# Cardinal-Cryptography/zk-apps

Hardware: AMD Instinct MI355X
Metric: shielder_withdraw_groth16_proofs_per_sec_2^20_constraints (higher is better)
Workload: dtype int: signed 28-bit limbs in 32-bit words, 64-bit column accumulators (Fr 255-bit / Fq 381-bit Montgomery); 1 GPU; single withdraw-shaped Groth16 proof, N=2^20 (7 Fr NTTs, 4 G1 MSM + 1 G2 MSM of 2^20-1 terms), 1 proof per step per GPU; relation=update_note (withdraw) with Poseidon-5 hashing, chain-padded to N, curve=BLS12-381, independent_proofs_per_rank=171, distinct_witnesses_per_rank=64, fresh_r_s_per_proof=True, proofs_in_flight_per_gpu=3, msm_schedule=A | B1 (over r*z) + L + H reduced together | B2 (G2)

## Files before the change

include/zkmi.h:

```cpp
#ifndef ZKMI_H
#define ZKMI_H
#include <stdint.h>
#ifdef __cplusplus
extern "C" {
#endif

#define ZKMI_OK 0
#define ZKMI_ERR_BAD_ARG (-1)
#define ZKMI_ERR_NON_CANONICAL (-2)
#define ZKMI_ERR_HIP (-3)
#define ZKMI_ERR_NO_DEVICE (-4)
#define ZKMI_ERR_VERIFICATION (-5)
#define ZKMI_ERR_ACCOUNT_UPDATE (-6)
#define ZKMI_ERR_OPERATION_COMBINE (-7)
#define ZKMI_ERR_UNSATISFIED (-8)
#define ZKMI_ERR_RCCL (-9)

typedef struct zkmi_ctx zkmi_ctx;
typedef struct zkmi_bases_g1 zkmi_bases_g1;
typedef struct zkmi_bases_g2 zkmi_bases_g2;
typedef struct zkmi_r1cs zkmi_r1cs;
typedef struct zkmi_pk zkmi_pk;

const char* zkmi_version(void);
// ... 145 lines not shown
#define ZKMI_OP_DEPOSIT 0
#define ZKMI_OP_WITHDRAW 1
#define ZKMI_MAX_TREE_HEIGHT 32
typedef struct {
  zkmi_fr amount, token, user;
  zkmi_fr new_note[3];
  zkmi_fr old_note[3];
  uint32_t tree_height;
  uint8_t path_shape[ZKMI_MAX_TREE_HEIGHT];
  zkmi_fr path[ZKMI_MAX_TREE_HEIGHT];
  zkmi_fr op_priv_user;
  zkmi_fr account[4];
} zkmi_note_update;
int32_t zkmi_update_note_r1cs(uint32_t log_n, int32_t op_kind, zkmi_r1cs** out);
int32_t zkmi_update_note_r1cs_h(uint32_t log_n, int32_t op_kind, uint32_t tree_height, zkmi_r1cs** out);
int32_t zkmi_update_note_witness(uint32_t log_n, int32_t op_kind, const zkmi_note_update* in, uint8_t* out_z,
                                 uint8_t* out_publics);

int32_t zkmi_update_note_witness_batch_dev(zkmi_ctx* ctx, uint32_t log_n, int32_t op_kind, const zkmi_note_update* in,
                                           uint32_t n, void* const* d_z_out, int32_t* out_status);
int32_t zkmi_update_note_witness_values_host(uint32_t log_n, int32_t op_kind, const zkmi_note_update* in, uint8_t* out_z);

int32_t zkmi_groth16_setup(zkmi_ctx* ctx, const zkmi_r1cs* r1cs, const uint8_t toxic[160], zkmi_pk** out_pk,
                           uint8_t* vk_out, uint64_t vk_cap);
int32_t zkmi_ctx_set_group_size(zkmi_ctx* ctx, uint32_t group);
int32_t zkmi_pk_load(zkmi_ctx* ctx, const zkmi_r1cs* r1cs, const uint8_t alpha_g1[96], const uint8_t beta_g1[96],
                     const uint8_t beta_g2[192], const uint8_t delta_g1[96], const uint8_t delta_g2[192],
                     const uint8_t* a_query, const uint8_t* b_g1_query, const uint8_t* b_g2_query,
                     const uint8_t* h_query, const uint8_t* l_query, zkmi_pk** out_pk);
int32_t zkmi_pk_free(zkmi_pk* pk);
int32_t zkmi_pk_shape(const zkmi_pk* pk, uint32_t* n_vars, uint32_t* n_pub, uint32_t* log_n);
int32_t zkmi_pk_export_g1_elems(const zkmi_pk* pk, uint8_t out_beta_g1[96], uint8_t out_delta_g1[96]);
int32_t zkmi_pk_schedule_state(const zkmi_pk* pk, uint64_t out[3]);
int32_t zkmi_pk_export_query(zkmi_ctx* ctx, const zkmi_pk* pk, int32_t which, uint64_t first, uint64_t count, uint8_t* out);
int32_t zkmi_groth16_prove(zkmi_ctx* ctx, const zkmi_pk* pk, const uint8_t* z, const uint8_t r[32], const uint8_t s[32],
                           uint8_t out_proof[192]);
int32_t zkmi_groth16_prove_dev(zkmi_ctx* ctx, const zkmi_pk* pk, const void* d_z, const uint8_t r[32], const uint8_t s[32],
                               uint8_t out_proof[192]);
int32_t zkmi_groth16_prove_batch_dev(zkmi_ctx* ctx, const zkmi_pk* pk, uint32_t n_proofs, const void* const* d_z,
                                     const uint8_t* r, const uint8_t* s, uint8_t* out_proofs);
int32_t zkmi_groth16_prove_batch(zkmi_ctx* ctx, const zkmi_pk* pk, uint32_t n_proofs, const uint8_t* const* z,
                                 const uint8_t* r, const uint8_t* s, uint8_t* out_proofs);
int32_t zkmi_groth16_witness_map(zkmi_ctx* ctx, const zkmi_pk* pk, const uint8_t* z, uint8_t* out_h);
int32_t zkmi_groth16_prove_batch_multi(zkmi_ctx* const* ctxs, const zkmi_pk* const* pks, uint32_t n_dev, uint32_t n_proofs,
                                       const void* const* z, int32_t z_on_device, const uint8_t* r, const uint8_t* s,
                                       uint8_t* out_proofs);

int32_t zkmi_groth16_verify(const uint8_t* vk, uint32_t n_pub, const uint8_t* publics, const uint8_t proof[192]);

typedef struct zkmi_vk zkmi_vk;
int32_t zkmi_vk_prepare(const uint8_t* vk, uint32_t n_pub, zkmi_vk** out);
int32_t zkmi_vk_free(zkmi_vk* vk);

#define ZKMI_PROOF_OK 0
#define ZKMI_PROOF_BAD_ENCODING 1
#define ZKMI_PROOF_NOT_ON_CURVE 2
#define ZKMI_PROOF_NOT_IN_SUBGROUP 3
#define ZKMI_PROOF_BAD_PUBLIC 4
#define ZKMI_PROOF_PAIRING 5
int32_t zkmi_groth16_verify_batch(zkmi_ctx* ctx, const zkmi_vk* vk, uint64_t n, const uint8_t* publics,
                                  const uint8_t* proofs, const uint8_t* weights, uint8_t* out_status,
                                  uint64_t* out_first_bad);
int32_t zkmi_groth16_verify_each(zkmi_ctx* ctx, const zkmi_vk* vk, uint64_t n, const uint8_t* publics,
                                 const uint8_t* proofs, uint8_t* out_status, uint64_t* out_first_bad);

int32_t zkmi_ark_vk_read(const uint8_t* buf, uint64_t len, int32_t compressed, uint8_t* out_vk, uint64_t vk_cap,
// ... 89 lines not shown
```

include/zkmi_testing.h:

```cpp
#ifndef ZKMI_TESTING_H
#define ZKMI_TESTING_H
#include "zkmi.h"
#ifdef __cplusplus
extern "C" {
#endif

int32_t zkmi_bases_g1_synthetic(zkmi_ctx* ctx, uint64_t n, zkmi_bases_g1** out);
int32_t zkmi_bases_g2_synthetic(zkmi_ctx* ctx, uint64_t n, zkmi_bases_g2** out);
int32_t zkmi_bases_g1_synthetic_range(zkmi_ctx* ctx, uint64_t first, uint64_t n, zkmi_bases_g1** out);
int32_t zkmi_bn254_bases_synthetic(zkmi_ctx* ctx, uint64_t n, zkmi_bn_bases** out);

int32_t zkmi_shielder_r1cs(uint32_t log_n, zkmi_r1cs** out);
int32_t zkmi_shielder_witness(uint32_t log_n, uint64_t seed, uint8_t* out_z );
int32_t zkmi_shielder_witness_from_input(uint32_t log_n, const zkmi_update_note_input* in, uint8_t* out_z);

int32_t zkmi_selftest_fq28(uint64_t seed, uint32_t iters, uint32_t* out_mismatches);
int32_t zkmi_selftest_assembly(uint64_t seed, uint32_t iters, uint32_t* out_mismatches);
int32_t zkmi_selftest_host_pool(uint32_t callers, uint32_t jobs, uint32_t* out_mismatches);
int32_t zkmi_selftest_poseidon(int32_t field, uint64_t seed, uint32_t iters, uint32_t* out_mismatches);
int32_t zkmi_selftest_miller_formulas(const uint8_t g1_affine[96], const uint8_t g2_affine[192], uint8_t out_fq12[576]);
int32_t zkmi_selftest_final_exp_formulas(const uint8_t in_fq12[576], uint8_t out_chain[576], uint8_t out_plain[576]);
int32_t zkmi_verify_each_kernel_ms(float out_ms[3]);
int32_t zkmi_verify_batch_phases(double out_ms[7]);
int32_t zkmi_selftest_quad_add(zkmi_ctx* ctx, uint64_t seed, uint32_t n, uint32_t* out_mismatches);
int32_t zkmi_selftest_fp28_ops(zkmi_ctx* ctx, int32_t field, int32_t op, uint32_t n, const int32_t* in, int32_t* out,
                               uint8_t* out_flag);
int32_t zkmi_selftest_ntt_dif_dev(zkmi_ctx* ctx, int32_t field, void* d_data, uint32_t log_n, int32_t post);
int32_t zkmi_selftest_msm_g1_sum2_dev(zkmi_ctx* ctx, const void* d_scalars_a, const void* d_scalars_b, uint64_t n,
                                      const zkmi_bases_g1* bases, uint8_t out_affine[96]);

#ifdef __cplusplus
}
#endif
#endif
```

zk-apps_amd/binding.py:

```python
import ctypes as C
import os

ERR = {
    0: "OK",
    -1: "BAD_ARG",
    -2: "NON_CANONICAL",
    -3: "HIP",
    -4: "NO_DEVICE",
    -5: "VerificationError",
    -6: "AccountUpdateError",
    -7: "OperationCombineError",
    -8: "UNSATISFIED",
    -9: "RCCL",
}
PHASES = {
    "msm_sort": 0,
    "msm_accum_g1": 1,
    "msm_reduce_g1": 2,
    "msm_accum_g2": 3,
    "msm_reduce_g2": 4,
    "ntt": 5,
    "witness": 6,
    "misc": 7,
}
# ... 1005 lines not shown
        self.ctx._chk(fn(self.ctx.h, self.h))
        return self

    def free(self):
        if self.h:
            fn = self.ctx.lib.zkmi_bases_g1_free if self.group == 1 else self.ctx.lib.zkmi_bases_g2_free
            fn(self.h)
            self.h = None


class ProvingKey:
    def __init__(self, ctx, h, r1cs):
        self.ctx, self.h, self.r1cs = ctx, h, r1cs

    def export_query(self, which, first, count):
        w = 192 if which == 2 else 96
        out = (C.c_uint8 * (w * count))()
        self.ctx._chk(self.ctx.lib.zkmi_pk_export_query(self.ctx.h, self.h, C.c_int32(which), C.c_uint64(first), C.c_uint64(count), out))
        return bytes(out)

    def check(self, checks=CHECK_SUBGROUP):
        where = (C.c_uint64 * 2)(NO_INDEX, NO_INDEX)
        rc = self.ctx.lib.zkmi_pk_check(self.ctx.h, self.h, C.c_int32(checks), where)
        if rc == -2:
            return int(where[0]), int(where[1])
        self.ctx._chk(rc)
        return None

    def schedule_state(self):
        out = (C.c_uint64 * 3)()
        self.ctx._chk(self.ctx.lib.zkmi_pk_schedule_state(self.h, out))
        return bool(out[0]), int(out[1]), int(out[2])

    def free(self):
        if self.h:
            self.ctx.lib.zkmi_pk_free(self.h)
            self.h = None
```

zk-apps_amd/csrc/field28_selftest.hip:

```cpp
#include "ctx.hpp"
#include "field28.hpp"
#include "ntt.hpp"

#ifdef ZKMI_TESTING
using namespace zkmi;

namespace {
enum Op : int {
  OP_ADD = 0, OP_SUB, OP_NEG, OP_DBL, OP_CARRY, OP_MUL, OP_SQR, OP_LAZY_MUL, OP_MSM, OP_X3, OP_SSUB_MUL, OP_IS_ZERO,
  OP_FROM_CANON, OP_TO_CANON, OP_INV,
  OP_FQ2_MUL = 15, OP_FQ2_SQR, OP_FQ2_MSM, OP_FQ2_X3,
  OP_P_MUL = 19, OP_P_SQR, OP_P_MSM, OP_P_SSUB, OP_P_IS_ZERO,
  OP_MUL_FIPS = 24, OP_SQR_FIPS, OP_FIPS2, OP_FIPS4,
  OP_COUNT
};
constexpr int N_IN[OP_COUNT] = {2, 2, 1, 1, 2, 2, 1, 4, 6, 3, 3, 1, 1, 1, 1, 4, 2, 8, 6, 4, 2, 8, 4, 2, 2, 1, 4, 8};
constexpr int N_OUT[OP_COUNT] = {1, 1, 1, 1, 1, 1, 1, 1, 1, 1, 2, 0, 1, 1, 1, 2, 2, 2, 2, 2, 2, 2, 4, 0, 1, 1, 1, 1};

template <class F>
ZK_HD F ld(const int32_t* p) {
  F r;
#pragma unroll
  for (int i = 0; i < F::NL; i++) r.l[i] = p[i];
  return r;
}
template <class F>
ZK_HD void st(int32_t* p, const F& v) {
#pragma unroll
  for (int i = 0; i < F::NL; i++) p[i] = v.l[i];
}

template <class P, int OP>
ZK_HD void op_body(const int32_t* in, int32_t* out, uint8_t* flag, uint32_t t) {
  using F = Fp28<P>;
  constexpr int NL = F::NL;
// ... 124 lines not shown
    if (e == hipSuccess && n_flag) e = hipMemcpyAsync(out_flag, d_flag, (size_t)n_flag * n, hipMemcpyDeviceToHost, ctx->stream);
    const hipError_t es = hipStreamSynchronize(ctx->stream);
    if (e == hipSuccess) e = es;
    (void)hipFree(d_in);
    (void)hipFree(d_out);
    (void)hipFree(d_flag);
    return e == hipSuccess ? ZKMI_OK : ctx->hip_fail(e, "fp28 ops self-test");
  }
}

#define ZK_OP_CASE(OP) \
  case OP: return run_op<P, OP>(ctx, n, in, out, out_flag);
template <class P>
int32_t dispatch(zkmi_ctx* ctx, int32_t op, uint32_t n, const int32_t* in, int32_t* out, uint8_t* out_flag) {
  switch (op) {
    ZK_OP_CASE(OP_ADD) ZK_OP_CASE(OP_SUB) ZK_OP_CASE(OP_NEG) ZK_OP_CASE(OP_DBL) ZK_OP_CASE(OP_CARRY) ZK_OP_CASE(OP_MUL)
    ZK_OP_CASE(OP_SQR) ZK_OP_CASE(OP_LAZY_MUL) ZK_OP_CASE(OP_MSM) ZK_OP_CASE(OP_X3) ZK_OP_CASE(OP_SSUB_MUL)
    ZK_OP_CASE(OP_IS_ZERO) ZK_OP_CASE(OP_FROM_CANON) ZK_OP_CASE(OP_TO_CANON) ZK_OP_CASE(OP_INV)
    ZK_OP_CASE(OP_MUL_FIPS) ZK_OP_CASE(OP_SQR_FIPS) ZK_OP_CASE(OP_FIPS2) ZK_OP_CASE(OP_FIPS4)
    default: break;
  }
  if constexpr (std::is_same<P, Fq28Params>::value) {
    switch (op) {
      ZK_OP_CASE(OP_FQ2_MUL) ZK_OP_CASE(OP_FQ2_SQR) ZK_OP_CASE(OP_FQ2_MSM) ZK_OP_CASE(OP_FQ2_X3)
      ZK_OP_CASE(OP_P_MUL) ZK_OP_CASE(OP_P_SQR) ZK_OP_CASE(OP_P_MSM) ZK_OP_CASE(OP_P_SSUB) ZK_OP_CASE(OP_P_IS_ZERO)
      default: break;
    }
  }
  return ZKMI_ERR_BAD_ARG;
}
#undef ZK_OP_CASE

template <class F, class Dom>
int32_t ntt_dif(zkmi_ctx* ctx, Dom* dom, void* d_data, uint32_t log_n, int32_t post) {
  const uint32_t n = 1u << log_n;
  const uint64_t bytes = (uint64_t)n * sizeof(F);
  if (ctx->d_work_cap < bytes) {
    if (ctx->d_work) (void)hipFree(ctx->d_work);
    ctx->d_work = nullptr;
    ctx->d_work_cap = 0;
    ZK_HIP(ctx, hipMalloc(&ctx->d_work, bytes));
    ctx->d_work_cap = bytes;
  }
  F* work = static_cast<F*>(ctx->d_work);
  ZK_HIP(ctx, ntt_from_canonical(static_cast<const uint32_t*>(d_data), work, n, ctx->stream));
  ZK_HIP(ctx, dom->inverse_to_rev(work, post ? dom->rev_coset_n : nullptr, nullptr, ctx->stream));
  ZK_HIP(ctx, ntt_to_canonical(work, static_cast<uint32_t*>(d_data), n, ctx->stream));
  ZK_HIP(ctx, hipStreamSynchronize(ctx->stream));
  return ZKMI_OK;
}
}

extern "C" int32_t zkmi_selftest_fp28_ops(zkmi_ctx* ctx, int32_t field, int32_t op, uint32_t n, const int32_t* in, int32_t* out,
                                          uint8_t* out_flag) {
  if (!in || n == 0 || n > (1u << 20) || op < 0 || op >= OP_COUNT) return ZKMI_ERR_BAD_ARG;
  switch (field) {
    case 0: return dispatch<Fq28Params>(ctx, op, n, in, out, out_flag);
    case 1: return dispatch<Fr28Params>(ctx, op, n, in, out, out_flag);
    case 2: return dispatch<BnFq28Params>(ctx, op, n, in, out, out_flag);
    case 3: return dispatch<BnFr28Params>(ctx, op, n, in, out, out_flag);
    default: return ZKMI_ERR_BAD_ARG;
  }
}

extern "C" int32_t zkmi_selftest_ntt_dif_dev(zkmi_ctx* ctx, int32_t field, void* d_data, uint32_t log_n, int32_t post) {
  ZK_ENTER(ctx);
  if (!d_data || log_n == 0 || log_n > 26 || (field != 1 && field != 3)) return ZKMI_ERR_BAD_ARG;
  hipError_t e;
  if (field == 1) {
    NttDomain* dom = ctx->domain((int)log_n, &e);
    if (!dom) return ctx->hip_fail(e, "ntt domain init");
    return ntt_dif<Fr28>(ctx, dom, d_data, log_n, post);
  }
  NttDomainBn* dom = ctx->domain_bn((int)log_n, &e);
  if (!dom) return ctx->hip_fail(e, "bn254 ntt domain init");
  return ntt_dif<BnFr28>(ctx, dom, d_data, log_n, post);
}
#endif
```

zk-apps_amd/csrc/groth16.hip:

```cpp
#include <stdlib.h>
#include <string.h>
#include <new>
#include <string>
#include <memory>
#include <chrono>
#include <functional>
#include <thread>
#include <vector>
#include "ctx.hpp"
#include "tune.hpp"
#include "host_pool.hpp"
#include "pairing.hpp"
#include "r1cs.hpp"
#include "points.hpp"

namespace zkmi {

template <class T>
__device__ __forceinline__ T ldv(const T* p) {
  T r;
  const uint4* s = reinterpret_cast<const uint4*>(p);
  uint4* d = reinterpret_cast<uint4*>(&r);
#pragma unroll
  for (unsigned i = 0; i < sizeof(T) / 16; i++) d[i] = s[i];
  return r;
}
template <class T>
__device__ __forceinline__ void stv(T* p, const T& v) {
  const uint4* s = reinterpret_cast<const uint4*>(&v);
  uint4* d = reinterpret_cast<uint4*>(p);
#pragma unroll
  for (unsigned i = 0; i < sizeof(T) / 16; i++) d[i] = s[i];
}

struct MatSet {
  const uint32_t* rowptr[3];
  const uint32_t* col[3];
  const Fr28* val[3];
};
constexpr uint32_t MATVEC_LONG_ROW = 1024;
__global__ void __launch_bounds__(256)
k_matvec_long(MatSet ms, const uint32_t* __restrict__ rows, const Fr28* __restrict__ z, Fr28* __restrict__ out_base, uint32_t n, uint32_t n_vars) {
  __shared__ Fr28 part[256];
  const uint32_t m = rows[2 * blockIdx.x], i = rows[2 * blockIdx.x + 1];
  const uint32_t* __restrict__ col = ms.col[m];
  const Fr28* __restrict__ val = ms.val[m];
  z += (size_t)blockIdx.y * n_vars;
  Fr28 acc = Fr28::zero();
  const uint32_t b = ms.rowptr[m][i], e = ms.rowptr[m][i + 1];
  for (uint32_t k = b + threadIdx.x; k < e; k += 256) acc = acc + ld28(val + k) * ld28(z + col[k]);
  part[threadIdx.x] = acc;
  __syncthreads();
  for (int o = 128; o > 0; o >>= 1) {
    if ((int)threadIdx.x < o) part[threadIdx.x] = part[threadIdx.x] + part[threadIdx.x + o];
    __syncthreads();
  }
  if (threadIdx.x == 0) st28(out_base + (size_t)m * gridDim.y * n + (size_t)blockIdx.y * n + i, part[0]);
}

template <int S>
__global__ void __launch_bounds__(256)
k_matvec(MatSet ms, const Fr28* __restrict__ z, Fr28* __restrict__ out_base, uint32_t nc, uint32_t n, uint32_t n_pub,
         uint32_t n_vars) {
  const int m = blockIdx.z;
  const uint32_t* __restrict__ rowptr = ms.rowptr[m];
  const uint32_t* __restrict__ col = ms.col[m];
  const Fr28* __restrict__ val = ms.val[m];
  const int is_a = m == 0;
  Fr28* __restrict__ out = out_base + (size_t)m * gridDim.y * n;
  z += (size_t)blockIdx.y * n_vars;
  out += (size_t)blockIdx.y * n;
  const uint32_t gi = blockIdx.x * blockDim.x + threadIdx.x;
  const uint32_t i = gi / S, lane = gi % S;
  if (i >= n) return;
  Fr28 acc = Fr28::zero();
  if (i < nc) {
    const uint32_t b = rowptr[i], e = rowptr[i + 1];
    if (e - b > MATVEC_LONG_ROW) return;
    for (uint32_t k = b + lane; k < e; k += S) acc = acc + ld28(val + k) * ld28(z + col[k]);
  } else if (is_a && i < nc + n_pub && lane == 0) {
    acc = ld28(z + (i - nc));
  }
  if constexpr (S > 1) {
#pragma unroll
    for (int o = S / 2; o > 0; o >>= 1) {
      Fr28 t;
#pragma unroll
      for (int q = 0; q < Fr28::NL; q++) t.l[q] = __shfl_xor(acc.l[q], o);
      acc = acc + t;
    }
    if (lane != 0) return;
  }
  st28(out + i, acc);
}

__global__ void __launch_bounds__(256)
k_check_sat(const Fr28* __restrict__ a, const Fr28* __restrict__ b, const Fr28* __restrict__ c,
            const Fr28* __restrict__ z, uint32_t nc, uint32_t* __restrict__ flag, uint32_t n, uint32_t n_vars) {
  a += (size_t)blockIdx.y * n;
  b += (size_t)blockIdx.y * n;
  c += (size_t)blockIdx.y * n;
  z += (size_t)blockIdx.y * n_vars;
  const uint32_t i = blockIdx.x * blockDim.x + threadIdx.x;
  bool bad = false;
  if (i < nc) {
    const Fr28 d = (ld28(a + i) * ld28(b + i) - ld28(c + i)) * Fr28::one();
    bad = !d.is_zero();
  }
  if (i == 0) {
    const Fr28 d = (ld28(z) - Fr28::one()) * Fr28::one();
    bad = bad || !d.is_zero();
  }
// ... 85 lines not shown
      Affine<F> p = ldv(table + w * 256 + d);
      acc.madd(p);
    }
  }
  stv(out + i, acc.to_affine());
}

}

using namespace zkmi;

static bool prover_sort_side() { return ZK_TUNE("ZKMI_SORT_SIDE", 0) == 1; }
static uint32_t prover_solo_max_log() {
  const int v = ZK_TUNE("ZKMI_SOLO_MAX_LOG", 19);
  return (uint32_t)(v < 0 ? 0 : v > 28 ? 28 : v);
}
static bool prover_aux_split() { return ZK_TUNE("ZKMI_AUX_SPLIT", 1) != 0; }

static bool same_bucket_set(const MsmPlan& a, const MsmPlan& b) {
  return a.shared == b.shared && a.c == b.c && a.nwin == b.nwin && a.nb == b.nb && a.seg_log == b.seg_log &&
         a.vec_parts == b.vec_parts && a.ndigits == b.ndigits;
}

struct zkmi_pk {
  zkmi_ctx* ctx = nullptr;
  int device = -1;
  uint32_t n_vars = 0, n_pub = 0, nc = 0, log_n = 0;
  uint32_t tree_height = 0;
  uint32_t gmax = 1;
  uint32_t* d_rowptr[3] = {nullptr, nullptr, nullptr};
  uint32_t* d_long_rows = nullptr;
  uint32_t n_long_rows = 0;
  uint32_t* d_col[3] = {nullptr, nullptr, nullptr};
  Fr28* d_val[3] = {nullptr, nullptr, nullptr};
  G1Affine *a_query = nullptr, *b_g1_query = nullptr, *h_query = nullptr, *l_query = nullptr;
  G2Affine* b_g2_query = nullptr;
  Affine<Fq28>*a28 = nullptr, *b1_28 = nullptr, *h28 = nullptr, *h28_rev = nullptr, *l28 = nullptr;
  Affine<Fq2_28>* b2_28 = nullptr;
  bool shared = false;
  Affine<Fq28>*a_tab = nullptr, *b1_tab = nullptr, *l_tab = nullptr, *h_tab = nullptr;
  Affine<Fq2_28>* b2_tab = nullptr;
  G1Affine alpha_g1, beta_g1, delta_g1, a0, b1_0;
  G2Affine beta_g2, delta_g2, b2_0;
  std::unique_ptr<FixedBase8<Fq>> delta1_tab, k1_tab;
  std::unique_ptr<FixedBase8<Fq2>> delta2_tab;
  G1Affine ka;
  G2Affine kb2;
  Fr* d_z[zkmi_ctx::PROOF_RING] = {};
  mutable const Fr* z_cur[zkmi_ctx::PROOF_RING] = {};
  uint32_t* d_rz[zkmi_ctx::PROOF_RING] = {};
  uint32_t* d_h[zkmi_ctx::PROOF_RING] = {};
  Fr28 *d_zm = nullptr, *d_a = nullptr;
  uint32_t* h_unsat = nullptr;
  uint32_t* h_zent = nullptr;
  mutable bool fold_dense = true;
  mutable uint64_t last_entries = 0, last_full = 0;
  ~zkmi_pk() {
    if (device >= 0) (void)hipSetDevice(device);
    (void)hipDeviceSynchronize();
    for (int m = 0; m < 3; m++) {
      if (d_rowptr[m]) (void)hipFree(d_rowptr[m]);
      if (d_col[m]) (void)hipFree(d_col[m]);
      if (d_val[m]) (void)hipFree(d_val[m]);
    }
    if (d_long_rows) (void)hipFree(d_long_rows);
    void* ptrs[] = {a_query, b_g1_query, h_query, l_query, b_g2_query, d_zm, d_a, a28, b1_28, h28, h28_rev, l28, b2_28,
// ... 9 lines not shown

static hipError_t pk_alloc(zkmi_pk* pk, zkmi_ctx* ctx, const zkmi_r1cs* r) {
  pk->ctx = ctx;
  pk->device = ctx->device;
  pk->n_vars = r->n_vars;
  pk->n_pub = r->n_pub;
  pk->nc = r->n_constraints;
  pk->log_n = r->log_n;
  pk->tree_height = r->tree_height;
  const uint64_t N = 1ull << r->log_n;
  hipError_t e;
  {
    std::vector<uint32_t> longs;
    for (uint32_t m = 0; m < 3; m++)
      for (uint32_t i = 0; i + 1 < r->m[m].rowptr.size(); i++)
        if (r->m[m].rowptr[i + 1] - r->m[m].rowptr[i] > MATVEC_LONG_ROW) {
          longs.push_back(m);
          longs.push_back(i);
        }
    pk->n_long_rows = (uint32_t)(longs.size() / 2);
    if (pk->n_long_rows) {
      if ((e = hipMalloc(&pk->d_long_rows, sizeof(uint32_t) * longs.size())) != hipSuccess) return e;
      if ((e = hipMemcpy(pk->d_long_rows, longs.data(), sizeof(uint32_t) * longs.size(), hipMemcpyHostToDevice)) != hipSuccess) return e;
    }
  }
  for (int m = 0; m < 3; m++) {
    const auto& c = r->m[m];
    const size_t nnz = c.col.size();
    if ((e = hipMalloc(&pk->d_rowptr[m], sizeof(uint32_t) * c.rowptr.size())) != hipSuccess) return e;
    if ((e = hipMalloc(&pk->d_col[m], sizeof(uint32_t) * (nnz ? nnz : 1))) != hipSuccess) return e;
    if ((e = hipMalloc(&pk->d_val[m], sizeof(Fr28) * (nnz ? nnz : 1))) != hipSuccess) return e;
    if ((e = hipMemcpy(pk->d_rowptr[m], c.rowptr.data(), sizeof(uint32_t) * c.rowptr.size(), hipMemcpyHostToDevice)) != hipSuccess) return e;
    if (nnz) {
      if ((e = hipMemcpy(pk->d_col[m], c.col.data(), sizeof(uint32_t) * nnz, hipMemcpyHostToDevice)) != hipSuccess) return e;
      std::vector<Fr> canon(nnz);
      for (size_t k = 0; k < nnz; k++) canon[k] = c.val[k].from_mont();
      if ((e = ctx->staging(sizeof(Fr) * nnz)) != hipSuccess) return e;
      if ((e = hipMemcpy(ctx->d_tmp, canon.data(), sizeof(Fr) * nnz, hipMemcpyHostToDevice)) != hipSuccess) return e;
      if ((e = ntt_from_canonical(static_cast<const uint32_t*>(ctx->d_tmp), pk->d_val[m], (uint32_t)nnz, ctx->stream)) != hipSuccess) return e;
      if ((e = hipStreamSynchronize(ctx->stream)) != hipSuccess) return e;
    }
  }
  if ((e = hipMalloc(&pk->a_query, sizeof(G1Affine) * r->n_vars)) != hipSuccess) return e;
  if ((e = hipMalloc(&pk->b_g1_query, sizeof(G1Affine) * r->n_vars)) != hipSuccess) return e;
  if ((e = hipMalloc(&pk->b_g2_query, sizeof(G2Affine) * r->n_vars)) != hipSuccess) return e;
  if ((e = hipMalloc(&pk->l_query, sizeof(G1Affine) * r->n_vars)) != hipSuccess) return e;
  if ((e = hipMalloc(&pk->h_query, sizeof(G1Affine) * N)) != hipSuccess) return e;
  if ((e = hipMalloc(&pk->a28, sizeof(Affine<Fq28>) * r->n_vars)) != hipSuccess) return e;
  if ((e = hipMalloc(&pk->b1_28, sizeof(Affine<Fq28>) * r->n_vars)) != hipSuccess) return e;
  if ((e = hipMalloc(&pk->b2_28, sizeof(Affine<Fq2_28>) * r->n_vars)) != hipSuccess) return e;
  if ((e = hipMalloc(&pk->l28, sizeof(Affine<Fq28>) * r->n_vars)) != hipSuccess) return e;
  if ((e = hipMalloc(&pk->h28, sizeof(Affine<Fq28>) * N)) != hipSuccess) return e;
  if ((e = hipMalloc(&pk->h28_rev, sizeof(Affine<Fq28>) * N)) != hipSuccess) return e;
  {
    uint32_t g = r->log_n <= 19 ? (1u << (r->log_n >= 14 ? 20 - r->log_n : 6)) : 1u;
    if (g > 64) g = 64;
    const uint32_t forced = ctx->group_override;
    if (forced >= 1 && forced <= 64 && (r->log_n <= 19 || forced == 1)) g = forced;
    const uint64_t capv = (1ull << r->log_n) > r->n_vars ? (1ull << r->log_n) : r->n_vars;
    const uint32_t parts = (uint32_t)msm_make_plan_shared(capv).nwin;
    while (g > 1 && g * parts > 64) g >>= 1;
    pk->gmax = g;
  }
  const uint64_t G = pk->gmax;
  for (int i = 0; i < zkmi_ctx::PROOF_RING; i++) {
    if ((e = hipMalloc(&pk->d_z[i], sizeof(Fr) * r->n_vars * G)) != hipSuccess) return e;
    if ((e = hipMalloc(&pk->d_h[i], 32ull * N * G)) != hipSuccess) return e;
// ... 369 lines not shown
    if (!sec[k].cnt) continue;
    uint64_t bad = UINT64_MAX;
    uint32_t st = 0;
    const int32_t rc = points_read(ctx, sec[k].group, sec[k].src, sec[k].cnt, PT_ENC_RESIDENT, checks, nullptr, false, nullptr, &bad, &st);
    if (rc != ZKMI_OK) return rc;
    if (bad != UINT64_MAX) {
      if (out_where) out_where[0] = (uint64_t)k, out_where[1] = bad;
      return ctx->fail(ZKMI_ERR_NON_CANONICAL, std::string("proving key: ") + PK_QUERY_NAME[k] + "[" + std::to_string(bad) +
                                                   "] (section " + std::to_string(k) + "): " + point_status_name(st));
    }
  }
  return ZKMI_OK;
}

int32_t zkmi_pk_free(zkmi_pk* pk) {
  if (!pk) return ZKMI_ERR_BAD_ARG;
  delete pk;
  return ZKMI_OK;
}

int32_t zkmi_pk_shape(const zkmi_pk* pk, uint32_t* n_vars, uint32_t* n_pub, uint32_t* log_n) {
  if (!pk) return ZKMI_ERR_BAD_ARG;
  if (n_vars) *n_vars = pk->n_vars;
  if (n_pub) *n_pub = pk->n_pub;
  if (log_n) *log_n = pk->log_n;
  return ZKMI_OK;
}

int32_t zkmi_pk_schedule_state(const zkmi_pk* pk, uint64_t out[3]) {
  if (!pk || !out) return ZKMI_ERR_BAD_ARG;
  out[0] = (pk->d_rz[0] != nullptr && pk->fold_dense) ? 1 : 0;
  out[1] = pk->last_entries;
  out[2] = pk->last_full;
  return ZKMI_OK;
}

int32_t zkmi_ctx_set_group_size(zkmi_ctx* ctx, uint32_t group) {
  if (!ctx || group > 64) return ZKMI_ERR_BAD_ARG;
  ctx->group_override = group;
  return ZKMI_OK;
}

int32_t zkmi_pk_export_g1_elems(const zkmi_pk* pk, uint8_t out_beta_g1[96], uint8_t out_delta_g1[96]) {
  if (!pk || !out_beta_g1 || !out_delta_g1) return ZKMI_ERR_BAD_ARG;
  g1_to_wire(pk->beta_g1, out_beta_g1);
  g1_to_wire(pk->delta_g1, out_delta_g1);
  return ZKMI_OK;
}

int32_t zkmi_pk_export_query(zkmi_ctx* ctx, const zkmi_pk* pk, int32_t which, uint64_t first, uint64_t count,
                             uint8_t* out) {
  ZK_ENTER(ctx);
  if (!ctx || !pk || !out || which < 0 || which > 4) return ZKMI_ERR_BAD_ARG;
  const uint64_t N = 1ull << pk->log_n;
  if (which == 2) {
    if (first + count > pk->n_vars) return ZKMI_ERR_BAD_ARG;
    std::vector<G2Affine> h(count);
    ZK_HIP(ctx, hipMemcpy(h.data(), pk->b_g2_query + first, sizeof(G2Affine) * count, hipMemcpyDeviceToHost));
    for (uint64_t i = 0; i < count; i++) g2_to_wire(h[i], out + 192 * i);
    return ZKMI_OK;
  }
  const G1Affine* src = which == 0 ? pk->a_query : which == 1 ? pk->b_g1_query : which == 3 ? pk->h_query : pk->l_query + pk->n_pub;
  const uint64_t len = which == 3 ? N - 1 : which == 4 ? pk->n_vars - pk->n_pub : pk->n_vars;
  if (first + count > len) return ZKMI_ERR_BAD_ARG;
  std::vector<G1Affine> h(count);
  ZK_HIP(ctx, hipMemcpy(h.data(), src + first, sizeof(G1Affine) * count, hipMemcpyDeviceToHost));
// ... 719 lines not shown
```

zk-apps_amd/csrc/ntt.hip:

```cpp
#include <stdlib.h>
#include <type_traits>
#include <utility>
#include "ntt.hpp"
#include "tune.hpp"

namespace zkmi {

namespace {

__device__ __forceinline__ void ld_words8(const uint32_t* p, uint32_t* w) {
  const uint4* q = reinterpret_cast<const uint4*>(p);
  const uint4 a = q[0], b = q[1];
  w[0] = a.x; w[1] = a.y; w[2] = a.z; w[3] = a.w;
  w[4] = b.x; w[5] = b.y; w[6] = b.z; w[7] = b.w;
}
__device__ __forceinline__ void st_words8(uint32_t* p, const uint32_t* w) {
  uint4* q = reinterpret_cast<uint4*>(p);
  q[0] = make_uint4(w[0], w[1], w[2], w[3]);
  q[1] = make_uint4(w[4], w[5], w[6], w[7]);
}

template <class F>
__global__ void k_bitrev_copy(const F* __restrict__ in, F* __restrict__ out, int log_n) {
  const uint32_t i = blockIdx.x * blockDim.x + threadIdx.x;
  if (i >= (1u << log_n)) return;
  const uint32_t r = log_n ? (__brev(i) >> (32 - log_n)) : 0u;
  st28(out + r, ld28(in + i));
}

template <class F, bool DIF, bool LOCAL_TW, int THREADS>
__global__ void __launch_bounds__(THREADS)
k_ntt_pass(F* __restrict__ data, const F* __restrict__ tw, int log_n, int t0, int S, int Q,
           const F* __restrict__ post, const F* __restrict__ sub, uint32_t* __restrict__ canon_out) {
  data += (size_t)blockIdx.y << log_n;
  if (sub) sub += (size_t)blockIdx.y << log_n;
  if (canon_out) canon_out += ((size_t)blockIdx.y << log_n) * 8;
  extern __shared__ __align__(16) unsigned char lds_raw[];
  F* tile = reinterpret_cast<F*>(lds_raw);
  const uint32_t tile_n = 1u << (S + Q);
  F* ctw = tile + tile_n;
  const uint32_t blk = blockIdx.x;
  const uint32_t mid_bits = (t0 > 0) ? (uint32_t)(t0 - Q) : 0u;
  const uint32_t mid = blk & ((1u << mid_bits) - 1u);
  const uint32_t hi = blk >> mid_bits;
  const uint32_t qeff = (t0 > 0) ? (uint32_t)Q : 0u;
  auto gindex = [&](uint32_t L) -> uint32_t {
    if (t0 == 0) return blk * tile_n + L;
    const uint32_t e = L >> Q, c = L & ((1u << Q) - 1u);
    return (hi << (t0 + S)) | (e << t0) | (mid << Q) | c;
  };
  auto twist = [&](uint32_t L) -> F {
    const uint32_t e = L >> Q, c = L & ((1u << Q) - 1u);
    const uint32_t col = (mid << Q) | c;
    const uint32_t ex = (col * (__brev(e) >> (32 - S))) << (log_n - t0 - S);
    const uint32_t halfn = 1u << (log_n - 1);
    F f = ld28(tw + (ex & (halfn - 1u)));
    return (ex & halfn) ? f.neg() : f;
  };
  if (LOCAL_TW)
    for (uint32_t k = threadIdx.x; k < (1u << (S - 1)); k += THREADS) ctw[k] = ld28(tw + ((size_t)k << (log_n - S)));
  for (uint32_t L = threadIdx.x; L < tile_n; L += THREADS) {
    F v = ld28(data + gindex(L));
    if (LOCAL_TW && !DIF && t0 > 0) v = v * twist(L);
    tile[L] = v;
  }
  __syncthreads();

  const uint32_t half = tile_n >> 1;
  for (int s = 0; s < S; s++) {
    const int u = DIF ? (S - 1 - s) : s;
    const int t = t0 + u;
    const uint32_t dist_log = (uint32_t)u + qeff;
    const uint32_t dist = 1u << dist_log;
    for (uint32_t b = threadIdx.x; b < half; b += THREADS) {
      const uint32_t lo = b & (dist - 1u);
      const uint32_t L0 = ((b >> dist_log) << (dist_log + 1)) | lo;
      const uint32_t L1 = L0 | dist;
      F w;
      if (LOCAL_TW) {
        w = ctw[(lo >> qeff) << (S - 1 - u)];
      } else {
        const uint32_t j = gindex(L0) & ((1u << t) - 1u);
        w = ld28(tw + ((size_t)j << (log_n - 1 - t)));
      }
      const F x = tile[L0];
      if (DIF) {
        const F y = tile[L1];
        tile[L0] = x + y;
        tile[L1] = x.sub_lazy(y) * w;
      } else {
        const F y = tile[L1] * w;
        tile[L0] = x + y;
        tile[L1] = x - y;
      }
    }
    __syncthreads();
  }

  for (uint32_t L = threadIdx.x; L < tile_n; L += THREADS) {
    const uint32_t g = gindex(L);
    F v = tile[L];
    if (LOCAL_TW && DIF && t0 > 0) v = v * twist(L);
    if (sub) v = v - ld28(sub + g);
    if (post) v = v * ld28(post + g);
    if (canon_out) {
      uint32_t w[8];
      v.to_canonical(w);
      st_words8(canon_out + (size_t)g * 8, w);
    } else {
      st28(data + g, v);
    }
  }
}

#ifdef ZKMI_EXPERIMENTS
#include "ntt_exp.hpp"
#endif

template <class F>
__global__ void __launch_bounds__(256)
k_mul_table(F* __restrict__ a, const F* __restrict__ b, uint32_t n) {
  const uint32_t i = blockIdx.x * blockDim.x + threadIdx.x;
  if (i < n) st28(a + i, ld28(a + i) * ld28(b + i));
}

template <class F>
__global__ void __launch_bounds__(256)
k_sub(F* __restrict__ a, const F* __restrict__ b, uint32_t n) {
  const uint32_t i = blockIdx.x * blockDim.x + threadIdx.x;
  if (i < n) st28(a + i, ld28(a + i) - ld28(b + i));
// ... 347 lines not shown
```

Baseline: 60.31 proofs/s.

## Specialize trivial-twiddle NTT stages as radix-4 and tag ±1 matvec coefficients

Inside the NTT tile kernel, the first two stages (DIT) or last two (DIF) whose twiddles are trivial run as one fused radix-4 step. It uses a single multiply by the 4th root of unity and lazy adds, and saves a shared-memory round trip and a barrier. Separately, the R1CS column indices now carry a 2-bit class marking coefficients equal to +1 or -1, so the sparse matvec uses an add or subtract instead of a field multiply for those terms. Risks are lazy-reduction headroom in the radix-4 path, which the added host-side reference with max-limb tracking is meant to check, and a limit of 2^30 columns.

```diff
diff --git a/include/zkmi.h b/include/zkmi.h
--- a/include/zkmi.h
+++ b/include/zkmi.h
@@ -201,6 +201,7 @@
 int32_t zkmi_pk_shape(const zkmi_pk* pk, uint32_t* n_vars, uint32_t* n_pub, uint32_t* log_n);
 int32_t zkmi_pk_export_g1_elems(const zkmi_pk* pk, uint8_t out_beta_g1[96], uint8_t out_delta_g1[96]);
 int32_t zkmi_pk_schedule_state(const zkmi_pk* pk, uint64_t out[3]);
+int32_t zkmi_pk_coef_classes(const zkmi_pk* pk, uint64_t out[3]);
 int32_t zkmi_pk_export_query(zkmi_ctx* ctx, const zkmi_pk* pk, int32_t which, uint64_t first, uint64_t count, uint8_t* out);
 int32_t zkmi_groth16_prove(zkmi_ctx* ctx, const zkmi_pk* pk, const uint8_t* z, const uint8_t r[32], const uint8_t s[32],
                            uint8_t out_proof[192]);
diff --git a/include/zkmi_testing.h b/include/zkmi_testing.h
--- a/include/zkmi_testing.h
+++ b/include/zkmi_testing.h
@@ -26,6 +26,9 @@
 int32_t zkmi_selftest_fp28_ops(zkmi_ctx* ctx, int32_t field, int32_t op, uint32_t n, const int32_t* in, int32_t* out,
                                uint8_t* out_flag);
 int32_t zkmi_selftest_ntt_dif_dev(zkmi_ctx* ctx, int32_t field, void* d_data, uint32_t log_n, int32_t post);
+int32_t zkmi_selftest_ntt_batch_dev(zkmi_ctx* ctx, int32_t field, void* d_data, uint32_t log_n, uint32_t batch, int32_t dif);
+int32_t zkmi_selftest_ntt_steps_host(int32_t field, uint32_t log_n, int32_t dif, const uint8_t pattern[64], uint8_t* out,
+                                     int64_t* out_max_top);
 int32_t zkmi_selftest_msm_g1_sum2_dev(zkmi_ctx* ctx, const void* d_scalars_a, const void* d_scalars_b, uint64_t n,
                                       const zkmi_bases_g1* bases, uint8_t out_affine[96]);
 
diff --git a/zk-apps_amd/binding.py b/zk-apps_amd/binding.py
--- a/zk-apps_amd/binding.py
+++ b/zk-apps_amd/binding.py
@@ -1061,6 +1061,11 @@
         self.ctx._chk(self.ctx.lib.zkmi_pk_schedule_state(self.h, out))
         return bool(out[0]), int(out[1]), int(out[2])
 
+    def coef_classes(self):
+        out = (C.c_uint64 * 3)()
+        self.ctx._chk(self.ctx.lib.zkmi_pk_coef_classes(self.h, out))
+        return int(out[0]), int(out[1]), int(out[2])
+
     def free(self):
         if self.h:
             self.ctx.lib.zkmi_pk_free(self.h)
diff --git a/zk-apps_amd/csrc/field28_selftest.hip b/zk-apps_amd/csrc/field28_selftest.hip
--- a/zk-apps_amd/csrc/field28_selftest.hip
+++ b/zk-apps_amd/csrc/field28_selftest.hip
@@ -1,6 +1,9 @@
 #include "ctx.hpp"
 #include "field28.hpp"
 #include "ntt.hpp"
+#include "ntt_butterfly.hpp"
+#include <string.h>
+#include <vector>
 
 #ifdef ZKMI_TESTING
 using namespace zkmi;
@@ -191,8 +194,8 @@
 #undef ZK_OP_CASE
 
 template <class F, class Dom>
-int32_t ntt_dif(zkmi_ctx* ctx, Dom* dom, void* d_data, uint32_t log_n, int32_t post) {
-  const uint32_t n = 1u << log_n;
+int32_t ntt_dif(zkmi_ctx* ctx, Dom* dom, void* d_data, uint32_t log_n, int32_t post, uint32_t batch = 1, bool dit = false) {
+  const uint32_t n = batch << log_n;
   const uint64_t bytes = (uint64_t)n * sizeof(F);
   if (ctx->d_work_cap < bytes) {
     if (ctx->d_work) (void)hipFree(ctx->d_work);
@@ -203,9 +206,106 @@
   }
   F* work = static_cast<F*>(ctx->d_work);
   ZK_HIP(ctx, ntt_from_canonical(static_cast<const uint32_t*>(d_data), work, n, ctx->stream));
-  ZK_HIP(ctx, dom->inverse_to_rev(work, post ? dom->rev_coset_n : nullptr, nullptr, ctx->stream));
+  if (dit) ZK_HIP(ctx, dom->forward_from_rev(work, ctx->stream, batch));
+  else ZK_HIP(ctx, dom->inverse_to_rev(work, post ? dom->rev_coset_n : nullptr, nullptr, ctx->stream, batch));
   ZK_HIP(ctx, ntt_to_canonical(work, static_cast<uint32_t*>(d_data), n, ctx->stream));
   ZK_HIP(ctx, hipStreamSynchronize(ctx->stream));
+  return ZKMI_OK;
+}
+
+template <class F>
+int32_t ntt_steps_host(uint32_t log_n, bool dif, const uint8_t* pattern, uint8_t* out, int64_t* out_max_top) {
+  using H = typename NttField<F>::Host;
+  const uint32_t n = 1u << log_n, halfn = n >> 1;
+  auto rev = [](uint32_t v, uint32_t bits) {
+    uint32_t r = 0;
+    for (uint32_t i = 0; i < bits; i++) r |= ((v >> i) & 1u) << (bits - 1 - i);
+    return r;
+  };
+  H w = NttField<F>::root_max();
+  for (int i = NttField<F>::TWO_ADICITY; i > (int)log_n; i--) w = w.sqr();
+  if (dif) w = w.inv();
+  const H wc = w.from_mont();
+  const F w28 = F::from_canonical(wc.l);
+  std::vector<F> tw(halfn), a(n);
+  tw[0] = F::one();
+  for (uint32_t k = 1; k < halfn; k++) tw[k] = tw[k - 1] * w28;
+  F pat[2];
+  for (int k = 0; k < 2; k++) {
+    uint32_t words[8];
+    memcpy(words, pattern + 32 * k, 32);
+    pat[k] = F::from_canonical(words);
+  }
+  for (uint32_t i = 0; i < n; i++) a[i] = pat[dif ? (i & 1u) : (i >> (log_n - 1))];
+  int64_t max_top = 0;
+  auto seen = [&](const F& v) {
+    const int64_t t = v.l[F::NL - 1] < 0 ? -(int64_t)v.l[F::NL - 1] : (int64_t)v.l[F::NL - 1];
+    if (t > max_top) max_top = t;
+  };
+  struct Pass {
+    uint32_t t0, S;
+  } passes[4];
+  int np = 0;
+  for (uint32_t t0 = 0; t0 < log_n; np++) {
+    const uint32_t S = log_n - t0 > 10 ? 10 : log_n - t0;
+    passes[np] = {t0, S};
+    t0 += S;
+  }
+  const bool local_tw = np <= 2;
+  for (int k = 0; k < np; k++) {
+    const uint32_t t0 = passes[dif ? np - 1 - k : k].t0, S = passes[dif ? np - 1 - k : k].S;
+    auto twist = [&](uint32_t g) {
+      const uint32_t e = (g >> t0) & ((1u << S) - 1u), col = g & ((1u << t0) - 1u);
+      const uint32_t ex = (col * rev(e, S)) << (log_n - t0 - S);
+      const F f = tw[ex & (halfn - 1u)];
+      a[g] = a[g] * ((ex & halfn) ? f.neg() : f);
+      seen(a[g]);
+    };
+    const bool trivial = local_tw || t0 == 0;
+    const uint32_t n_trivial = !trivial ? 0u : (S >= 2 ? 2u : 1u);
+    auto trivial_stages = [&]() {
+      const uint32_t d = 1u << t0;
+      if (S >= 2) {
+        const F w4 = tw[1u << (log_n - 2)];
+        for (uint32_t g = 0; g < n; g++) {
+          if (g & (3u * d)) continue;
+          if (dif) ntt_dif_tail4(a[g], a[g + d], a[g + 2 * d], a[g + 3 * d], w4);
+          else ntt_dit_head4(a[g], a[g + d], a[g + 2 * d], a[g + 3 * d], w4);
+          for (uint32_t q = 0; q < 4; q++) seen(a[g + q * d]);
+        }
+      } else {
+        for (uint32_t g = 0; g < n; g++) {
+          if (g & d) continue;
+          ntt_butterfly_unit(a[g], a[g + d]);
+          seen(a[g]), seen(a[g + d]);
+        }
+      }
+    };
+    if (!dif && local_tw && t0 > 0)
+      for (uint32_t g = 0; g < n; g++) twist(g);
+    if (!dif && trivial) trivial_stages();
+    for (uint32_t s = 0; s < S - n_trivial; s++) {
+      const uint32_t u = dif ? S - 1 - s : s + n_trivial, t = t0 + u, dist = 1u << t;
+      for (uint32_t g = 0; g < n; g++) {
+        if (g & dist) continue;
+        F wv;
+        if (local_tw) wv = tw[(size_t)(((g >> t0) & ((1u << u) - 1u)) << (S - 1 - u)) << (log_n - S)];
+        else wv = tw[(size_t)(g & (dist - 1u)) << (log_n - 1 - t)];
+        if (dif) ntt_dif_butterfly(a[g], a[g + dist], wv);
+        else ntt_dit_butterfly(a[g], a[g + dist], wv);
+        seen(a[g]), seen(a[g + dist]);
+      }
+    }
+    if (dif && trivial) trivial_stages();
+    if (dif && local_tw && t0 > 0)
+      for (uint32_t g = 0; g < n; g++) twist(g);
+  }
+  for (uint32_t i = 0; i < n; i++) {
+    uint32_t words[8];
+    a[dif ? rev(i, log_n) : i].to_canonical(words);
+    memcpy(out + 32ull * i, words, 32);
+  }
+  *out_max_top = max_top;
   return ZKMI_OK;
 }
 }
@@ -235,4 +335,25 @@
   if (!dom) return ctx->hip_fail(e, "bn254 ntt domain init");
   return ntt_dif<BnFr28>(ctx, dom, d_data, log_n, post);
 }
+
+extern "C" int32_t zkmi_selftest_ntt_batch_dev(zkmi_ctx* ctx, int32_t field, void* d_data, uint32_t log_n, uint32_t batch, int32_t dif) {
+  ZK_ENTER(ctx);
+  if (!d_data || log_n == 0 || log_n > 20 || batch == 0 || batch > 64 || (field != 1 && field != 3)) return ZKMI_ERR_BAD_ARG;
+  hipError_t e;
+  if (field == 1) {
+    NttDomain* dom = ctx->domain((int)log_n, &e);
+    if (!dom) return ctx->hip_fail(e, "ntt domain init");
+    return ntt_dif<Fr28>(ctx, dom, d_data, log_n, 0, batch, dif == 0);
+  }
+  NttDomainBn* dom = ctx->domain_bn((int)log_n, &e);
+  if (!dom) return ctx->hip_fail(e, "bn254 ntt domain init");
+  return ntt_dif<BnFr28>(ctx, dom, d_data, log_n, 0, batch, dif == 0);
+}
+
+extern "C" int32_t zkmi_selftest_ntt_steps_host(int32_t field, uint32_t log_n, int32_t dif, const uint8_t pattern[64], uint8_t* out,
+                                                int64_t* out_max_top) {
+  if (!pattern || !out || !out_max_top || log_n == 0 || log_n > 24 || (field != 1 && field != 3)) return ZKMI_ERR_BAD_ARG;
+  return field == 1 ? ntt_steps_host<Fr28>(log_n, dif != 0, pattern, out, out_max_top)
+                    : ntt_steps_host<BnFr28>(log_n, dif != 0, pattern, out, out_max_top);
+}
 #endif
diff --git a/zk-apps_amd/csrc/groth16.hip b/zk-apps_amd/csrc/groth16.hip
--- a/zk-apps_amd/csrc/groth16.hip
+++ b/zk-apps_amd/csrc/groth16.hip
@@ -39,6 +39,15 @@
   const Fr28* val[3];
 };
 constexpr uint32_t MATVEC_LONG_ROW = 1024;
+constexpr uint32_t COL_CLASS_SHIFT = 30, COL_INDEX_MASK = (1u << COL_CLASS_SHIFT) - 1u;
+constexpr uint32_t COL_PLUS_ONE = 1u, COL_MINUS_ONE = 2u;
+__device__ __forceinline__ Fr28 matvec_term(const Fr28& acc, uint32_t ck, const Fr28* __restrict__ val, uint32_t k, const Fr28* __restrict__ z) {
+  const Fr28 zv = ld28(z + (ck & COL_INDEX_MASK));
+  const uint32_t cls = ck >> COL_CLASS_SHIFT;
+  if (cls == COL_PLUS_ONE) return acc + zv;
+  if (cls == COL_MINUS_ONE) return acc - zv;
+  return acc + ld28(val + k) * zv;
+}
 __global__ void __launch_bounds__(256)
 k_matvec_long(MatSet ms, const uint32_t* __restrict__ rows, const Fr28* __restrict__ z, Fr28* __restrict__ out_base, uint32_t n, uint32_t n_vars) {
   __shared__ Fr28 part[256];
@@ -48,7 +57,7 @@
   z += (size_t)blockIdx.y * n_vars;
   Fr28 acc = Fr28::zero();
   const uint32_t b = ms.rowptr[m][i], e = ms.rowptr[m][i + 1];
-  for (uint32_t k = b + threadIdx.x; k < e; k += 256) acc = acc + ld28(val + k) * ld28(z + col[k]);
+  for (uint32_t k = b + threadIdx.x; k < e; k += 256) acc = matvec_term(acc, col[k], val, k, z);
   part[threadIdx.x] = acc;
   __syncthreads();
   for (int o = 128; o > 0; o >>= 1) {
@@ -77,7 +86,7 @@
   if (i < nc) {
     const uint32_t b = rowptr[i], e = rowptr[i + 1];
     if (e - b > MATVEC_LONG_ROW) return;
-    for (uint32_t k = b + lane; k < e; k += S) acc = acc + ld28(val + k) * ld28(z + col[k]);
+    for (uint32_t k = b + lane; k < e; k += S) acc = matvec_term(acc, col[k], val, k, z);
   } else if (is_a && i < nc + n_pub && lane == 0) {
     acc = ld28(z + (i - nc));
   }
@@ -229,6 +238,7 @@
   uint32_t* d_long_rows = nullptr;
   uint32_t n_long_rows = 0;
   uint32_t* d_col[3] = {nullptr, nullptr, nullptr};
+  uint64_t n_coef_class[3] = {0, 0, 0};
   Fr28* d_val[3] = {nullptr, nullptr, nullptr};
   G1Affine *a_query = nullptr, *b_g1_query = nullptr, *h_query = nullptr, *l_query = nullptr;
   G2Affine* b_g2_query = nullptr;
@@ -304,7 +314,15 @@
     if ((e = hipMalloc(&pk->d_val[m], sizeof(Fr28) * (nnz ? nnz : 1))) != hipSuccess) return e;
     if ((e = hipMemcpy(pk->d_rowptr[m], c.rowptr.data(), sizeof(uint32_t) * c.rowptr.size(), hipMemcpyHostToDevice)) != hipSuccess) return e;
     if (nnz) {
-      if ((e = hipMemcpy(pk->d_col[m], c.col.data(), sizeof(uint32_t) * nnz, hipMemcpyHostToDevice)) != hipSuccess) return e;
+      const Fr one = Fr::one(), minus_one = Fr::zero() - Fr::one();
+      std::vector<uint32_t> tagged(nnz);
+      for (size_t k = 0; k < nnz; k++) {
+        if (c.col[k] > COL_INDEX_MASK) return hipErrorInvalidValue;
+        const uint32_t cls = c.val[k] == one ? COL_PLUS_ONE : c.val[k] == minus_one ? COL_MINUS_ONE : 0u;
+        pk->n_coef_class[cls]++;
+        tagged[k] = c.col[k] | (cls << COL_CLASS_SHIFT);
+      }
+      if ((e = hipMemcpy(pk->d_col[m], tagged.data(), sizeof(uint32_t) * nnz, hipMemcpyHostToDevice)) != hipSuccess) return e;
       std::vector<Fr> canon(nnz);
       for (size_t k = 0; k < nnz; k++) canon[k] = c.val[k].from_mont();
       if ((e = ctx->staging(sizeof(Fr) * nnz)) != hipSuccess) return e;
@@ -740,6 +758,12 @@
   out[0] = (pk->d_rz[0] != nullptr && pk->fold_dense) ? 1 : 0;
   out[1] = pk->last_entries;
   out[2] = pk->last_full;
+  return ZKMI_OK;
+}
+
+int32_t zkmi_pk_coef_classes(const zkmi_pk* pk, uint64_t out[3]) {
+  if (!pk || !out) return ZKMI_ERR_BAD_ARG;
+  for (int i = 0; i < 3; i++) out[i] = pk->n_coef_class[i];
   return ZKMI_OK;
 }
 
diff --git a/zk-apps_amd/csrc/ntt.hip b/zk-apps_amd/csrc/ntt.hip
--- a/zk-apps_amd/csrc/ntt.hip
+++ b/zk-apps_amd/csrc/ntt.hip
@@ -2,6 +2,7 @@
 #include <type_traits>
 #include <utility>
 #include "ntt.hpp"
+#include "ntt_butterfly.hpp"
 #include "tune.hpp"
 
 namespace zkmi {
@@ -67,8 +68,43 @@
   __syncthreads();
 
   const uint32_t half = tile_n >> 1;
-  for (int s = 0; s < S; s++) {
-    const int u = DIF ? (S - 1 - s) : s;
+  const bool trivial = LOCAL_TW || t0 == 0;
+  const int n_trivial = !trivial ? 0 : (S >= 2 ? 2 : 1);
+  auto trivial_stages = [&]() {
+    const uint32_t d = 1u << qeff;
+    if (S >= 2) {
+      const F w4 = LOCAL_TW ? ctw[1u << (S - 2)] : ld28(tw + ((size_t)1 << (log_n - 2)));
+      for (uint32_t q = threadIdx.x; q < (tile_n >> 2); q += THREADS) {
+        const uint32_t L = ((q >> qeff) << (qeff + 2)) | (q & (d - 1u));
+        const uint32_t Lp = L + (DIF ? d : 2 * d), Lq = L + 3 * d;
+        const uint32_t Lr = L, Ls = L + (DIF ? 2 * d : d);
+        F xp = tile[Lp], xq = tile[Lq];
+        ntt_r4_product_half(xp, xq, w4);
+        __builtin_amdgcn_sched_barrier(0);
+        F xr = tile[Lr], xs = tile[Ls];
+        ntt_r4_lazy_half(xr, xs);
+        ntt_butterfly_unit(xr, xp);
+        tile[Lr] = xr;
+        tile[Lp] = xp;
+        __builtin_amdgcn_sched_barrier(0);
+        ntt_butterfly_unit(xs, xq);
+        tile[Ls] = xs;
+        tile[Lq] = xq;
+      }
+    } else {
+      for (uint32_t b = threadIdx.x; b < half; b += THREADS) {
+        const uint32_t L = ((b >> qeff) << (qeff + 1)) | (b & (d - 1u));
+        F x = tile[L], y = tile[L + d];
+        ntt_butterfly_unit(x, y);
+        tile[L] = x;
+        tile[L + d] = y;
+      }
+    }
+    __syncthreads();
+  };
+  if (!DIF && trivial) trivial_stages();
+  for (int s = 0; s < S - n_trivial; s++) {
+    const int u = DIF ? (S - 1 - s) : s + n_trivial;
     const int t = t0 + u;
     const uint32_t dist_log = (uint32_t)u + qeff;
     const uint32_t dist = 1u << dist_log;
@@ -83,19 +119,15 @@
         const uint32_t j = gindex(L0) & ((1u << t) - 1u);
         w = ld28(tw + ((size_t)j << (log_n - 1 - t)));
       }
-      const F x = tile[L0];
-      if (DIF) {
-        const F y = tile[L1];
-        tile[L0] = x + y;
-        tile[L1] = x.sub_lazy(y) * w;
-      } else {
-        const F y = tile[L1] * w;
-        tile[L0] = x + y;
-        tile[L1] = x - y;
-      }
+      F x = tile[L0], y = tile[L1];
+      if (DIF) ntt_dif_butterfly(x, y, w);
+      else ntt_dit_butterfly(x, y, w);
+      tile[L0] = x;
+      tile[L1] = y;
     }
     __syncthreads();
   }
+  if (DIF && trivial) trivial_stages();
 
   for (uint32_t L = threadIdx.x; L < tile_n; L += THREADS) {
     const uint32_t g = gindex(L);
diff --git a/zk-apps_amd/csrc/ntt_butterfly.hpp b/zk-apps_amd/csrc/ntt_butterfly.hpp
--- /dev/null
+++ b/zk-apps_amd/csrc/ntt_butterfly.hpp
@@ -0,0 +1,52 @@
+#pragma once
+#include "field28.hpp"
+
+namespace zkmi {
+
+template <class F>
+ZK_HD void ntt_dit_butterfly(F& x, F& y, const F& w) {
+  const F t = y * w;
+  y = x - t;
+  x = x + t;
+}
+template <class F>
+ZK_HD void ntt_dif_butterfly(F& x, F& y, const F& w) {
+  const F t = x.sub_lazy(y) * w;
+  x = x + y;
+  y = t;
+}
+template <class F>
+ZK_HD void ntt_butterfly_unit(F& x, F& y) {
+  const F t = x - y;
+  x = x + y;
+  y = t;
+}
+
+template <class F>
+ZK_HD void ntt_r4_product_half(F& p, F& q, const F& w4) {
+  const F t = p.sub_lazy(q);
+  p = p.add_lazy(q);
+  q = t * w4;
+}
+template <class F>
+ZK_HD void ntt_r4_lazy_half(F& p, F& q) {
+  const F t = p.sub_lazy(q);
+  p = p.add_lazy(q);
+  q = t;
+}
+template <class F>
+ZK_HD void ntt_dit_head4(F& x0, F& x1, F& x2, F& x3, const F& w4) {
+  ntt_r4_product_half(x2, x3, w4);
+  ntt_r4_lazy_half(x0, x1);
+  ntt_butterfly_unit(x0, x2);
+  ntt_butterfly_unit(x1, x3);
+}
+template <class F>
+ZK_HD void ntt_dif_tail4(F& x0, F& x1, F& x2, F& x3, const F& w4) {
+  ntt_r4_product_half(x1, x3, w4);
+  ntt_r4_lazy_half(x0, x2);
+  ntt_butterfly_unit(x0, x1);
+  ntt_butterfly_unit(x2, x3);
+}
+
+}
```

After: 60.05 proofs/s. Within noise of the previous version (-0.4%).
